# Desperodoo/distributed_multi_agent_reinforcement_learning

Hardware: AMD Instinct MI355X
Metric: env-steps/sec (whole node), pursuit-evasion 8-agent 4096-env (higher is better)
Workload: dtype f64 environment / f32 policy (f32 matrix products evaluated from exact 3-way bf16 operand splits, f32 accumulation and storage)

## Files before the change

distributed_multi_agent_reinforcement_learning_amd/csrc/mappo_split.hip:

```cpp
#include <hip/hip_runtime.h>
#include <stdint.h>
#include <string.h>

#include "mappo_ops.h"
#include "sb_gemm.hpp"
#include "sb_gru_seq.hpp"

extern "C" {

static int sb_gemm_any(int64_t R, int32_t N, int32_t K, const float *X, int64_t ldx, const float *W, int64_t ldw, const float *bias, int32_t relu,
                       const float *addend, int64_t lda, float *Y, int64_t ldy, uint8_t *ybits, int64_t ldyb, void *stream) {
    if (R < 0 || !X || !W || !Y || ldx < K || ldw < K || ldy < N || (addend && lda < N)) return MO_ERR_BAD_ARG;
    if ((ldx & 3) || (ldw & 3) || (ldy & 3) || (lda & 3) || ((uintptr_t)X & 15) || ((uintptr_t)W & 15) || ((uintptr_t)Y & 15) || ((uintptr_t)addend & 15) ||
        ((uintptr_t)bias & 15))
        return MO_ERR_BAD_ARG;
    if (R == 0) return 0;
    hipStream_t st = (hipStream_t)stream;
    if (N == 128 && K == 128) return launch_sb_gemm_best<4, 1>(R, X, ldx, W, ldw, bias, addend, lda, Y, ldy, relu, st, ybits, ldyb);
    if (N == 128 && K == 256) return launch_sb_gemm_best<8, 1>(R, X, ldx, W, ldw, bias, addend, lda, Y, ldy, relu, st, ybits, ldyb);
    if (ybits) return MO_ERR_BAD_ARG;
    if (N == 128 && K == 384) return launch_sb_gemm_best<12, 1>(R, X, ldx, W, ldw, bias, addend, lda, Y, ldy, relu, st);
    if (N == 256 && K == 128) return launch_sb_gemm_best<4, 2>(R, X, ldx, W, ldw, bias, addend, lda, Y, ldy, relu, st);
    if (N == 384 && K == 128) return launch_sb_gemm_best<4, 3>(R, X, ldx, W, ldw, bias, addend, lda, Y, ldy, relu, st);
    return MO_ERR_BAD_ARG;
}

int sb_gemm(int64_t R, int32_t N, int32_t K, const float *X, int64_t ldx, const float *W, int64_t ldw, const float *bias, int32_t relu,
            const float *addend, int64_t lda, float *Y, int64_t ldy, void *stream) {
    return sb_gemm_any(R, N, K, X, ldx, W, ldw, bias, relu, addend, lda, Y, ldy, nullptr, 0, stream);
}

int sb_gemm_signs(int64_t R, int32_t N, int32_t K, const float *X, int64_t ldx, const float *W, int64_t ldw, const float *bias, int32_t relu,
                  const float *addend, int64_t lda, float *Y, int64_t ldy, uint8_t *y_sign_bits, int64_t ld_bytes, void *stream) {
    if (!y_sign_bits || ld_bytes < N / 8) return MO_ERR_BAD_ARG;
    return sb_gemm_any(R, N, K, X, ldx, W, ldw, bias, relu, addend, lda, Y, ldy, y_sign_bits, ld_bytes, stream);
}

int64_t sb_gemm_masked_workspace(int32_t N) { return N > 0 ? (int64_t)1024 * N * 4 : 0; }

int sb_gemm_masked(int64_t R, int32_t N, int32_t K, const float *X, int64_t ldx, const float *W, int64_t ldw, const float *M, int64_t ldm,
                   int32_t mask_cols, float *Y, int64_t ldy, float *colsum, void *workspace, void *stream) {
    if (R < 0 || !X || !W || !M || !Y || !colsum || !workspace || ldx < K || ldw < K || ldy < N || ldm < N) return MO_ERR_BAD_ARG;
    if (mask_cols < 0 || mask_cols > N || (mask_cols & 127)) return MO_ERR_BAD_ARG;
    if ((ldx & 3) || (ldw & 3) || (ldy & 3) || (ldm & 3) || ((uintptr_t)X & 15) || ((uintptr_t)W & 15) || ((uintptr_t)Y & 15) || ((uintptr_t)M & 15) ||
        ((uintptr_t)colsum & 15) || ((uintptr_t)workspace & 15))
        return MO_ERR_BAD_ARG;
    hipStream_t st = (hipStream_t)stream;
    if (R == 0) return (int)hipMemsetAsync(colsum, 0, (size_t)N * 4, st);
    int dev = 0, cus = 256;
    if (hipGetDevice(&dev) == hipSuccess && hipDeviceGetAttribute(&cus, hipDeviceAttributeMultiprocessorCount, dev) != hipSuccess) cus = 256;
    if (cus > 512) return MO_ERR_BAD_ARG;
    float *part = (float *)workspace;
    const int mt = mask_cols / 128;
    if (N == 256 && K == 128) return launch_sb_gemm<4, 2, SBG_MASK_OPT_256>(R, X, ldx, W, ldw, nullptr, M, ldm, Y, ldy, 0, st, mt, part, colsum);
    if (N == 384 && K == 128) return launch_sb_gemm<4, 3, SBG_MASK_OPT_384>(R, X, ldx, W, ldw, nullptr, M, ldm, Y, ldy, 0, st, mt, part, colsum);
    if (N == 128 && K == 384) return launch_sb_gemm<12, 1, SBG_MASK_OPT_K384>(R, X, ldx, W, ldw, nullptr, M, ldm, Y, ldy, 0, st, mt, part, colsum);
    return MO_ERR_BAD_ARG;
}

int sb_gemm_masked_bits(int64_t R, int32_t N, int32_t K, const float *X, int64_t ldx, const float *W, int64_t ldw, const uint8_t *sign_bits,
                        int64_t ld_bytes, int32_t mask_cols, float *Y, int64_t ldy, float *colsum, void *workspace, void *stream) {
    if (R < 0 || !X || !W || !sign_bits || !Y || !colsum || !workspace || ldx < K || ldw < K || ldy < N || ld_bytes < N / 8) return MO_ERR_BAD_ARG;
    if (mask_cols < 0 || mask_cols > N || (mask_cols & 127)) return MO_ERR_BAD_ARG;
    if ((ldx & 3) || (ldw & 3) || (ldy & 3) || ((uintptr_t)X & 15) || ((uintptr_t)W & 15) || ((uintptr_t)Y & 15) || ((uintptr_t)colsum & 15) ||
        ((uintptr_t)workspace & 15))
        return MO_ERR_BAD_ARG;
    hipStream_t st = (hipStream_t)stream;
    if (R == 0) return (int)hipMemsetAsync(colsum, 0, (size_t)N * 4, st);
    int dev = 0, cus = 256;
    if (hipGetDevice(&dev) == hipSuccess && hipDeviceGetAttribute(&cus, hipDeviceAttributeMultiprocessorCount, dev) != hipSuccess) cus = 256;
    if (cus > 512) return MO_ERR_BAD_ARG;
    float *part = (float *)workspace;
    const float *m = (const float *)sign_bits;
    const int mt = mask_cols / 128;
    if (N == 256 && K == 128) return launch_sb_gemm<4, 2, SBG_MASK_OPT_256 | 16>(R, X, ldx, W, ldw, nullptr, m, ld_bytes, Y, ldy, 0, st, mt, part, colsum);
    if (N == 384 && K == 128) return launch_sb_gemm<4, 3, SBG_MASK_OPT_384 | 16>(R, X, ldx, W, ldw, nullptr, m, ld_bytes, Y, ldy, 0, st, mt, part, colsum);
    if (N == 128 && K == 384) return launch_sb_gemm<12, 1, SBG_MASK_OPT_K384 | 16>(R, X, ldx, W, ldw, nullptr, m, ld_bytes, Y, ldy, 0, st, mt, part, colsum);
    return MO_ERR_BAD_ARG;
}

int sb_gemm_n128(int64_t R, int32_t K, const float *X, int64_t ldx, const float *W, int64_t ldw, const float *bias, int32_t relu, const float *addend,
                 int64_t lda, float *Y, int64_t ldy, void *stream) {
    return sb_gemm(R, 128, K, X, ldx, W, ldw, bias, relu, addend, lda, Y, ldy, stream);
}

int gru_seq_split_fwd_multi(int32_t n_nets, const mo_gru_seq_net *nets, int32_t T, int32_t B, int32_t H, int32_t gi_agents, void *stream) {
    if (n_nets < 1 || n_nets > MO_GRU_MAX_NETS || !nets || T < 1 || B < 1 || H != SBR_H || gi_agents < 0 || (gi_agents && B % gi_agents)) return MO_ERR_BAD_ARG;
    for (int k = 0; k < n_nets; k++) {
        const mo_gru_seq_net &m = nets[k];
        if (!m.gi || !m.w_hh || !m.b_hh || !m.h0 || !m.out) return MO_ERR_BAD_ARG;
        if ((((uintptr_t)m.gi | (uintptr_t)m.w_hh | (uintptr_t)m.b_hh | (uintptr_t)m.h0 | (uintptr_t)m.out | (uintptr_t)m.save) & 15)) return MO_ERR_BAD_ARG;
        if (m.B < 0 || m.B > B || (gi_agents && m.B % gi_agents)) return MO_ERR_BAD_ARG;
    }
    return launch_gru_seq_fwd_sb(n_nets, nets, T, B, gi_agents, (hipStream_t)stream);
}

int gru_seq_split_bwd_multi(int32_t n_nets, const mo_gru_seq_bwd_net *nets, int32_t T, int32_t B, int32_t H, int32_t gi_agents, void *stream) {
    if (n_nets < 1 || n_nets > MO_GRU_MAX_NETS || !nets || T < 1 || B < 1 || H != SBR_H || gi_agents < 0 || (gi_agents && B % gi_agents)) return MO_ERR_BAD_ARG;
    for (int k = 0; k < n_nets; k++) {
        const mo_gru_seq_bwd_net &m = nets[k];
        if (!m.dout || !m.save || !m.out || !m.h0 || !m.w_hh || !m.dgi || !m.dh0) return MO_ERR_BAD_ARG;
        if ((m.dgh == nullptr) == (m.dnr == nullptr)) return MO_ERR_BAD_ARG;
        if ((m.db_ih || m.db_hh) && (!m.db_ih || !m.db_hh || !m.workspace)) return MO_ERR_BAD_ARG;
        if ((((uintptr_t)m.dout | (uintptr_t)m.save | (uintptr_t)m.out | (uintptr_t)m.h0 | (uintptr_t)m.dgi | (uintptr_t)m.dgh | (uintptr_t)m.dnr |
              (uintptr_t)m.dh0 | (uintptr_t)m.workspace) & 15)) return MO_ERR_BAD_ARG;
        if (m.B < 0 || m.B > B || (gi_agents && m.B % gi_agents)) return MO_ERR_BAD_ARG;
    }
    return launch_gru_seq_bwd_sb(n_nets, nets, T, B, gi_agents, (hipStream_t)stream);
}

}
```

include/mappo_ops.h:

```cpp
#ifndef MAPPO_OPS_H
#define MAPPO_OPS_H
#include <stdint.h>

#ifdef __cplusplus
extern "C" {
#endif

#define MO_ERR_BAD_ARG 20001

enum { MO_ADJ_TENSOR = 0,
       MO_ADJ_ONES = 1,
       MO_ADJ_VALID = 2,
       MO_ADJ_BITS = 3 };
#define MO_ADJ_ROW_WORDS(K) (((((K) + 31) >> 5) + 3) & ~3)

int dhgn_msg_agg_fwd(int32_t R, int32_t P, int32_t K, int32_t E, int32_t din, const float *p, int64_t p_row_stride,
                     const float *q, int64_t q_row_stride, int32_t q_div, const float *e, int64_t e_row_stride, const void *adj,
                     int64_t adj_row_stride, int32_t adj_mode, const int32_t *kvalid, const float *W, const float *b,
                     float *out, int64_t out_stride , void *stream);

typedef struct mo_msg_rel {
    int32_t K, din, q_div, adj_mode;
    const float *q; int64_t q_rs;
    const float *e; int64_t e_rs;
    const void *adj; int64_t adj_rs;
    const int32_t *kvalid;
    const float *W, *b;
} mo_msg_rel;
int dhgn_msg_agg3_fwd(const mo_msg_rel *rel , int32_t R, int32_t P, int32_t E, const float *p, int64_t p_row_stride, float *out,
                      int64_t out_stride, void *stream);
int dhgn_msg_agg3_pair_fwd(const mo_msg_rel *rel , int32_t R, int32_t P, int32_t E, const float *p, int64_t p_row_stride,
                           const int32_t *o_kvalid, float *out_actor, float *out_critic, int64_t out_stride, void *stream);

int dhgn_msg_agg3_pair01_fwd(const mo_msg_rel *rel , int32_t R, int32_t P, int32_t E, const float *p, int64_t p_row_stride,
                             float *out_actor, float *out_critic, int64_t out_stride, void *stream);
int dhgn_msg_agg_bwd_pair(int32_t R, int32_t P, int32_t K, int32_t E, int32_t din, const float *p, int64_t p_row_stride, const float *q,
                          int64_t q_row_stride, int32_t q_div, const float *e, int64_t e_row_stride, const float *adj, int64_t adj_row_stride,
                          const float *W, const float *b, const float *gout_actor, const float *gout_critic, int64_t gout_stride, float *dW,
                          float *db, void *workspace, void *stream);
int dhgn_msg_agg3_pair_pos_fwd(const mo_msg_rel *rel , int32_t R, int32_t P, int32_t E, const float *p, int64_t p_row_stride,
                               const int32_t *o_kvalid, float *out_actor, float *out_critic, int64_t out_stride, const float *Wp,
                               int64_t wp_row_stride, const float *bp, float *pos_actor, float *pos_critic, int64_t pos_stride, void *stream);

int64_t dhgn_msg_agg_bwd_workspace(int32_t E, int32_t din);
int dhgn_msg_agg_bwd(int32_t R, int32_t P, int32_t K, int32_t E, int32_t din, const float *p, int64_t p_row_stride,
                     const float *q, int64_t q_row_stride, int32_t q_div, const float *e, int64_t e_row_stride, const void *adj,
                     int64_t adj_row_stride, int32_t adj_mode, const int32_t *kvalid, const float *W, const float *b,
                     const float *gout, int64_t gout_stride, float *dW, float *db, void *workspace, void *stream);

int dhgn_msg_agg_ones_sorted_ok(int32_t R, int32_t P, int32_t K, int32_t E, int32_t din, int32_t q_div);
int64_t dhgn_msg_agg_ones_sorted_workspace(int32_t R, int32_t P, int32_t K, int32_t E, int32_t q_div, int64_t *m_bytes, int64_t *qtab_bytes,
                                           int64_t *partial_bytes);
int dhgn_msg_agg_ones_sorted_fwd(int32_t R, int32_t P, int32_t K, int32_t E, const float *p, int64_t p_row_stride, const float *q,
                                 int64_t q_row_stride, int32_t q_div, const float *W, const float *b, float *out, int64_t out_stride,
                                 uint8_t *save_m, float *qtab, void *stream);
int dhgn_msg_agg_ones_sorted_bwd(int32_t R, int32_t P, int32_t K, int32_t E, const float *p, int64_t p_row_stride, int32_t q_div,
                                 const float *gout, int64_t gout_stride, const uint8_t *save_m, const float *qtab, float *dW, float *db,
                                 void *partials, void *stream);

int64_t gae_advnorm_workspace(void);
int gae_advnorm(int32_t N, int32_t T, int32_t P, const float *r, const float *v, const float *active, float gamma,
                float lamda, int32_t use_adv_norm, float *adv, float *v_target, double *stats, void *stream);

int categorical_sample(int32_t R, int32_t A, const float *probs, uint64_t seed, uint64_t offset, int32_t greedy,
                       int32_t *action, float *logp, void *stream);
int categorical_sample_counter(int32_t R, int32_t A, const float *probs, uint64_t seed, uint64_t *counter, int32_t greedy,
                               int32_t *action, float *logp, void *stream);

int spectral_norm_weight(int32_t A, int32_t H, const float *W, float *u, float *v, float eps, int32_t n_power_iterations, float *w_eff,
                         void *stream);

int head_linear(int32_t R, int32_t A, int32_t H, const float *feat, const float *W, const float *b, float *y, void *stream);
int head_sample(int32_t R, int32_t A, int32_t H, const float *feat, const float *W, const float *b, uint64_t seed, uint64_t *counter,
                uint32_t *ticket, int32_t greedy, int32_t *action, float *logp, void *stream);

int gru_gates_fwd(int32_t B, int32_t H, const float *gi, const float *gh, const float *b_hh, const float *h_prev, float *h_out,
                  float *save, void *stream);
int gru_gates_bwd(int32_t B, int32_t H, const float *dout, const float *dcarry, const float *save, const float *h_prev, float *dgi,
                  float *dgh, float *dh_direct, void *stream);

int64_t gru_seq_save_elems(int32_t T, int32_t B);
#define MO_GRU_MAX_NETS 24
#define MO_GRU_CELL_MAX_NETS 4
typedef struct mo_gru_seq_net { const float *gi, *w_hh, *b_hh, *h0; float *out, *save; int32_t B, pad0; } mo_gru_seq_net;
typedef struct mo_gru_seq_bwd_net {
    const float *dout, *save, *out, *h0, *w_hh;
    float *dgi, *dgh, *dnr, *dh0, *db_ih, *db_hh;
    void *workspace;
    int32_t B, pad0;
} mo_gru_seq_bwd_net;
int gru_seq_fwd_multi(int32_t n_nets, const mo_gru_seq_net *nets, int32_t T, int32_t B, int32_t H, int32_t gi_agents, void *stream);
int gru_seq_bwd_multi(int32_t n_nets, const mo_gru_seq_bwd_net *nets, int32_t T, int32_t B, int32_t H, int32_t gi_agents, void *stream);
int gru_seq_split_fwd_multi(int32_t n_nets, const mo_gru_seq_net *nets, int32_t T, int32_t B, int32_t H, int32_t gi_agents, void *stream);
int gru_seq_split_bwd_multi(int32_t n_nets, const mo_gru_seq_bwd_net *nets, int32_t T, int32_t B, int32_t H, int32_t gi_agents, void *stream);
int gru_seq_fwd(int32_t T, int32_t B, int32_t H, const float *gi, const float *w_hh, const float *b_hh, const float *h0, float *out,
                float *save, int32_t gi_agents, void *stream);
int64_t gru_seq_bwd_workspace(int32_t B);
int gru_seq_bwd(int32_t T, int32_t B, int32_t H, const float *dout, const float *save, const float *out, const float *h0,
                const float *w_hh, float *dgi, float *dgh, float *dnr, float *dh0, float *db_ih, float *db_hh, int32_t gi_agents,
                void *workspace, void *stream);

int gru_cell_fwd(int32_t B, int32_t H, const float *x, const float *h_prev, const float *w_ih, const float *w_hh, const float *b_ih,
                 const float *b_hh, float *h_out, void *stream);
typedef struct mo_gru_cell_net { const float *x, *h_prev, *w_ih, *w_hh, *b_ih, *b_hh; float *h_out; } mo_gru_cell_net;
int gru_cell_fwd_multi(int32_t n_nets, const mo_gru_cell_net *nets, int32_t B, int32_t H, void *stream);
int gru_cell_split_fwd_multi(int32_t n_nets, const mo_gru_cell_net *nets, int32_t B, int32_t H, void *stream);
int sb_gemm_n128(int64_t R, int32_t K, const float *X, int64_t ldx, const float *W, int64_t ldw, const float *bias, int32_t relu, const float *C,
                 int64_t ldc, float *Y, int64_t ldy, void *stream);
int sb_gemm(int64_t R, int32_t N, int32_t K, const float *X, int64_t ldx, const float *W, int64_t ldw, const float *bias, int32_t relu, const float *C,
            int64_t ldc, float *Y, int64_t ldy, void *stream);
int sb_gemm_signs(int64_t R, int32_t N, int32_t K, const float *X, int64_t ldx, const float *W, int64_t ldw, const float *bias, int32_t relu, const float *C,
                  int64_t ldc, float *Y, int64_t ldy, uint8_t *y_sign_bits, int64_t ld_bytes, void *stream);
int64_t sb_gemm_masked_workspace(int32_t N);
int sb_gemm_masked(int64_t R, int32_t N, int32_t K, const float *X, int64_t ldx, const float *W, int64_t ldw, const float *M, int64_t ldm,
                   int32_t mask_cols, float *Y, int64_t ldy, float *colsum, void *workspace, void *stream);
int sb_gemm_masked_bits(int64_t R, int32_t N, int32_t K, const float *X, int64_t ldx, const float *W, int64_t ldw, const uint8_t *sign_bits,
                        int64_t ld_bytes, int32_t mask_cols, float *Y, int64_t ldy, float *colsum, void *workspace, void *stream);

int64_t ppo_loss_workspace(void);
int ppo_loss_fwd_bwd(int64_t n, const float *logp_now, const float *entropy, const float *logp_old, const float *adv, const float *active,
                     const float *values_now, const float *values_old, const float *v_target, const float *active_sum, float epsilon,
                     float entropy_coef, int32_t use_value_clip, float *losses, float *grad_logp, float *grad_entropy, float *grad_values,
                     void *workspace, void *stream);
int ppo_loss_prob_fwd_bwd(int64_t n, int32_t A, const float *prob, float *grad_prob, int64_t d1, int64_t d2, int64_t p_s0, int64_t p_s1, int64_t p_s2,
                          const float *action, const float *logp_old, const float *adv, const float *active, const float *values_now, int64_t v_s0,
                          int64_t v_s1, int64_t v_s2, const float *values_old, const float *v_target, const float *active_sum, float epsilon,
                          float entropy_coef, int32_t use_value_clip, float *losses, float *grad_values, void *workspace, void *stream);

int gauss_head_sample(int32_t R, int32_t A, int32_t H, const float *feat, const float *W, const float *b, const float *log_std, uint64_t seed,
                      uint64_t *counter, uint32_t *ticket, int32_t greedy, float *action, double *env_action, float *logp, void *stream);
int64_t ppo_loss_gauss_workspace(void);
int ppo_loss_gauss_fwd_bwd(int64_t n, int32_t A, const float *mu, float *grad_mu, int64_t d1, int64_t d2, int64_t m_s0, int64_t m_s1, int64_t m_s2,
                           const float *log_std, const float *action, const float *logp_old, const float *adv, const float *active,
                           const float *values_now, int64_t v_s0, int64_t v_s1, int64_t v_s2, const float *values_old, const float *v_target,
                           const float *active_sum, float epsilon, float entropy_coef, int32_t use_value_clip, float *losses, float *grad_values,
                           float *grad_log_std, void *workspace, void *stream);

#define MO_RECORD_MAX_ITEMS 16
typedef struct {
    const void *src;
    void *dst;
    int64_t dst_row_stride;
    int32_t row_bytes;
    int32_t i32_to_f32;
} mo_record_item;
int rollout_record(int32_t N, int32_t n_items, const mo_record_item *items, const float *raw, float *episode_return, int32_t P, void *stream);

int64_t wgrad_tn_workspace(int32_t M, int32_t N);
int wgrad_tn(int64_t K, int32_t M, int32_t N, const float *A, int64_t lda, const float *B, int64_t ldb, float *C, int32_t accumulate,
             void *workspace, void *stream);
int64_t wgrad_split_workspace(int32_t M, int32_t N);
int wgrad_split_tn(int64_t K, int32_t M, int32_t N, const float *A, int64_t lda, const float *B, int64_t ldb, float *C, int32_t accumulate,
                   void *workspace, void *stream);
int wgrad_split_tn2(int64_t K, int32_t M1, int32_t M2, int32_t N, const float *A1, int64_t lda1, const float *A2, int64_t lda2, const float *B, int64_t ldb,
                    float *C, int32_t accumulate, void *workspace, void *stream);
int fcra_neighbour_mean(int32_t R, int32_t P, int32_t E, int32_t T, const float *z_actor, int64_t za_episode_stride, int64_t za_step_stride,
                        const float *z_critic, int64_t zc_episode_stride, int64_t zc_step_stride, const float *adj, int64_t adj_row_stride,
                        const float *bias, int32_t relu, float *out_actor, float *out_critic, int64_t out_stride, void *stream);
#define MO_NBR_MAX_JOBS 4
typedef struct mo_nbr_job { const float *z_actor, *z_critic, *bias; float *out_actor, *out_critic; } mo_nbr_job;
int fcra_neighbour_mean_multi(int32_t n_jobs, const mo_nbr_job *jobs, int32_t R, int32_t P, int32_t E, int32_t T, int64_t za_episode_stride,
                              int64_t za_step_stride, int64_t zc_episode_stride, int64_t zc_step_stride, const float *adj, int64_t adj_row_stride,
                              int32_t relu, int64_t out_stride, void *stream);

int64_t relu_bwd_colsum_workspace(int32_t F);
int relu_bwd_colsum(int64_t R, int32_t F, const float *gout, int64_t g_row_stride, const float *y, int64_t y_row_stride, float *gin, float *colsum,
                    void *workspace, void *stream);

int64_t wgrad_skinny_workspace(int32_t NS, int32_t F);
int wgrad_skinny(int64_t R, int32_t NS, int32_t F, const float *S, int64_t lds, const float *X, int64_t ldx, int32_t transposed, float *C,
                 float *colsum_x, float *colsum_s, void *workspace, void *stream);

const char *mappo_ops_error_string(int code);

#ifdef __cplusplus
}
#endif
#endif
```

Measured before the change: 2.639 million.

## Add weight-stationary 32-row bf16-split GEMM kernel for masked 384-wide shapes

Adds a new persistent GEMM kernel that keeps the split bf16 weights in registers and streams 32-row input tiles through double-buffered shared memory, prefetching the next tile while the MFMAs run. It is enabled by default only for the masked (float-mask) 384-wide GEMMs at large row counts; other paths need an explicit selector call. The aim is to cut weight reloads and hide input latency, at the cost of high register pressure and a separate colsum reduction launch.

Result: no change. 2.638 million, median of 6 (-0.0%).

```diff
diff --git a/distributed_multi_agent_reinforcement_learning_amd/csrc/mappo_split.hip b/distributed_multi_agent_reinforcement_learning_amd/csrc/mappo_split.hip
--- a/distributed_multi_agent_reinforcement_learning_amd/csrc/mappo_split.hip
+++ b/distributed_multi_agent_reinforcement_learning_amd/csrc/mappo_split.hip
@@ -4,9 +4,20 @@
 
 #include "mappo_ops.h"
 #include "sb_gemm.hpp"
+#include "sb_gemm_w32.hpp"
 #include "sb_gru_seq.hpp"
 
+static constexpr int64_t SBW_MIN_ROWS = 131072;
+static int g_sbg_kernel = 0;
+static bool sbg_w32(int64_t R, bool by_default) { return g_sbg_kernel == 2 || (g_sbg_kernel == 0 && by_default && R >= SBW_MIN_ROWS); }
+
 extern "C" {
+
+int sb_gemm_select_kernel(int32_t which) {
+    if (which < 0 || which > 2) return MO_ERR_BAD_ARG;
+    g_sbg_kernel = which;
+    return 0;
+}
 
 static int sb_gemm_any(int64_t R, int32_t N, int32_t K, const float *X, int64_t ldx, const float *W, int64_t ldw, const float *bias, int32_t relu,
                        const float *addend, int64_t lda, float *Y, int64_t ldy, uint8_t *ybits, int64_t ldyb, void *stream) {
@@ -19,9 +30,17 @@
     if (N == 128 && K == 128) return launch_sb_gemm_best<4, 1>(R, X, ldx, W, ldw, bias, addend, lda, Y, ldy, relu, st, ybits, ldyb);
     if (N == 128 && K == 256) return launch_sb_gemm_best<8, 1>(R, X, ldx, W, ldw, bias, addend, lda, Y, ldy, relu, st, ybits, ldyb);
     if (ybits) return MO_ERR_BAD_ARG;
-    if (N == 128 && K == 384) return launch_sb_gemm_best<12, 1>(R, X, ldx, W, ldw, bias, addend, lda, Y, ldy, relu, st);
+    if (N == 128 && K == 384) {
+        if (sbg_w32(R, false)) return addend ? launch_sb_gemm_w32<12, 1, 1>(R, X, ldx, W, ldw, bias, addend, lda, Y, ldy, relu, st)
+                                      : launch_sb_gemm_w32<12, 1, 0>(R, X, ldx, W, ldw, bias, addend, lda, Y, ldy, relu, st);
+        return launch_sb_gemm_best<12, 1>(R, X, ldx, W, ldw, bias, addend, lda, Y, ldy, relu, st);
+    }
     if (N == 256 && K == 128) return launch_sb_gemm_best<4, 2>(R, X, ldx, W, ldw, bias, addend, lda, Y, ldy, relu, st);
-    if (N == 384 && K == 128) return launch_sb_gemm_best<4, 3>(R, X, ldx, W, ldw, bias, addend, lda, Y, ldy, relu, st);
+    if (N == 384 && K == 128) {
+        if (sbg_w32(R, false)) return addend ? launch_sb_gemm_w32<4, 3, 1>(R, X, ldx, W, ldw, bias, addend, lda, Y, ldy, relu, st)
+                                      : launch_sb_gemm_w32<4, 3, 0>(R, X, ldx, W, ldw, bias, addend, lda, Y, ldy, relu, st);
+        return launch_sb_gemm_best<4, 3>(R, X, ldx, W, ldw, bias, addend, lda, Y, ldy, relu, st);
+    }
     return MO_ERR_BAD_ARG;
 }
 
@@ -53,6 +72,10 @@
     float *part = (float *)workspace;
     const int mt = mask_cols / 128;
     if (N == 256 && K == 128) return launch_sb_gemm<4, 2, SBG_MASK_OPT_256>(R, X, ldx, W, ldw, nullptr, M, ldm, Y, ldy, 0, st, mt, part, colsum);
+    if (sbg_w32(R, true)) {
+        if (N == 384 && K == 128) return launch_sb_gemm_w32<4, 3, 4>(R, X, ldx, W, ldw, nullptr, M, ldm, Y, ldy, 0, st, mt, part, colsum);
+        if (N == 128 && K == 384) return launch_sb_gemm_w32<12, 1, 5>(R, X, ldx, W, ldw, nullptr, M, ldm, Y, ldy, 0, st, mt, part, colsum);
+    }
     if (N == 384 && K == 128) return launch_sb_gemm<4, 3, SBG_MASK_OPT_384>(R, X, ldx, W, ldw, nullptr, M, ldm, Y, ldy, 0, st, mt, part, colsum);
     if (N == 128 && K == 384) return launch_sb_gemm<12, 1, SBG_MASK_OPT_K384>(R, X, ldx, W, ldw, nullptr, M, ldm, Y, ldy, 0, st, mt, part, colsum);
     return MO_ERR_BAD_ARG;
@@ -74,6 +97,10 @@
     const float *m = (const float *)sign_bits;
     const int mt = mask_cols / 128;
     if (N == 256 && K == 128) return launch_sb_gemm<4, 2, SBG_MASK_OPT_256 | 16>(R, X, ldx, W, ldw, nullptr, m, ld_bytes, Y, ldy, 0, st, mt, part, colsum);
+    if (sbg_w32(R, false)) {
+        if (N == 384 && K == 128) return launch_sb_gemm_w32<4, 3, 20>(R, X, ldx, W, ldw, nullptr, m, ld_bytes, Y, ldy, 0, st, mt, part, colsum);
+        if (N == 128 && K == 384) return launch_sb_gemm_w32<12, 1, 20>(R, X, ldx, W, ldw, nullptr, m, ld_bytes, Y, ldy, 0, st, mt, part, colsum);
+    }
     if (N == 384 && K == 128) return launch_sb_gemm<4, 3, SBG_MASK_OPT_384 | 16>(R, X, ldx, W, ldw, nullptr, m, ld_bytes, Y, ldy, 0, st, mt, part, colsum);
     if (N == 128 && K == 384) return launch_sb_gemm<12, 1, SBG_MASK_OPT_K384 | 16>(R, X, ldx, W, ldw, nullptr, m, ld_bytes, Y, ldy, 0, st, mt, part, colsum);
     return MO_ERR_BAD_ARG;
diff --git a/distributed_multi_agent_reinforcement_learning_amd/csrc/sb_gemm_w32.hpp b/distributed_multi_agent_reinforcement_learning_amd/csrc/sb_gemm_w32.hpp
--- /dev/null
+++ b/distributed_multi_agent_reinforcement_learning_amd/csrc/sb_gemm_w32.hpp
@@ -0,0 +1,185 @@
+#pragma once
+#include <mutex>
+
+#include "sb_gemm.hpp"
+
+template <int KC, int NT, int OPT>
+__global__ __launch_bounds__(256) void k_sb_gemm_w32(int64_t R, const float *__restrict__ X, int64_t ldx, const float *__restrict__ W, int64_t ldw,
+                                                     const float *__restrict__ bias, const float *addend, int64_t lda, float *Y, int64_t ldy, int relu,
+                                                     int mask_tiles, float *__restrict__ colsum_part) {
+    static_assert(KC % 2 == 0 && KC * NT == 12, "the 384-wide shapes: 12 x 1 or 4 x 3");
+    extern __shared__ uint4 sbw_tile[];
+    constexpr int IMG = 3 * KC * 2 * 64, UPW = KC / 2, TPW = 2 * NT;
+    constexpr bool MASK = OPT & 4, BITS = (OPT & 4) && (OPT & 16), EARLY = (OPT & 1) && !BITS;
+    const int tid = threadIdx.x, w = tid >> 6, l = tid & 63, i = l & 15, gq = l >> 4;
+    uint4 wg[TPW][KC][3];
+#pragma unroll
+    for (int s = 0; s < TPW; s++) {
+        const float *rw = W + (size_t)(16 * (TPW * w + s) + i) * ldw + 8 * gq;
+#pragma unroll
+        for (int c = 0; c < KC; c++) sb_split8(*(const float4 *)(rw + 32 * c), *(const float4 *)(rw + 32 * c + 4), wg[s][c]);
+    }
+    const int64_t n_it = (R + 31) / 32;
+    float4 pf[UPW][2];
+    auto fetch1 = [&](int n, int64_t it) {
+        const int blk = w * UPW + n, c = blk >> 1, rt = blk & 1;
+        int64_t row = it * 32 + rt * 16 + i;
+        row = row < R ? row : R - 1;
+        const float *src = X + row * ldx + 32 * c + 8 * gq;
+        if constexpr (SBG_ABLATE & 4) {
+            pf[n][0] = pf[n][1] = make_float4((float)row * 1e-6f, 0.5f, -0.25f, (float)c);
+        } else {
+            pf[n][0] = *(const float4 *)src;
+            pf[n][1] = *(const float4 *)(src + 4);
+        }
+    };
+    auto stage1 = [&](int n, uint4 *img) {
+        const int blk = w * UPW + n;
+        uint4 p_[3];
+        sb_split8(pf[n][0], pf[n][1], p_);
+#pragma unroll
+        for (int p = 0; p < 3; p++) img[(p * KC * 2 + blk) * 64 + l] = p_[p];
+    };
+    int64_t it = blockIdx.x;
+#pragma unroll
+    for (int n = 0; n < UPW; n++) fetch1(n, it);
+#pragma unroll
+    for (int n = 0; n < UPW; n++) stage1(n, sbw_tile);
+#pragma unroll
+    for (int n = 0; n < UPW; n++) fetch1(n, it + gridDim.x);
+    lds_barrier();
+    int cur = 0;
+    float4 cs[TPW];
+#pragma unroll
+    for (int s = 0; s < TPW; s++) cs[s] = make_float4(0.f, 0.f, 0.f, 0.f);
+    for (; it < n_it; it += gridDim.x) {
+        const uint4 *tb = sbw_tile + cur * IMG + l;
+        uint4 *nimg = sbw_tile + (cur ^ 1) * IMG;
+        float4 a4[TPW][2];
+        unsigned mb[TPW][2];
+        if constexpr (EARLY) {
+#pragma unroll
+            for (int rt = 0; rt < 2; rt++) {
+                int64_t row = it * 32 + rt * 16 + i;
+                row = row < R ? row : R - 1;
+#pragma unroll
+                for (int s = 0; s < TPW; s++) a4[s][rt] = *(const float4 *)(addend + row * lda + 16 * (TPW * w + s) + 4 * gq);
+            }
+        }
+        f32x4 acc[TPW][2];
+#pragma unroll
+        for (int s = 0; s < TPW; s++) acc[s][0] = acc[s][1] = (f32x4){0.f, 0.f, 0.f, 0.f};
+        uint4 nb0[3], nb1[3];
+#pragma unroll
+        for (int p = 0; p < 3; p++) { nb0[p] = tb[(p * KC * 2) * 64]; nb1[p] = tb[(p * KC * 2 + 1) * 64]; }
+#pragma unroll
+        for (int c = 0; c < KC; c++) {
+            uint4 b0[3], b1[3];
+#pragma unroll
+            for (int p = 0; p < 3; p++) { b0[p] = nb0[p]; b1[p] = nb1[p]; }
+            if (c + 1 < KC) {
+#pragma unroll
+                for (int p = 0; p < 3; p++) { nb0[p] = tb[(p * KC * 2 + 2 * c + 2) * 64]; nb1[p] = tb[(p * KC * 2 + 2 * c + 3) * 64]; }
+            }
+            __builtin_amdgcn_sched_barrier(0);
+#define SBW_MMA(pi, pj)                                                                                                                             \
+            _Pragma("unroll") for (int s = 0; s < TPW; s++) {                                                                                         \
+                acc[s][0] = __builtin_amdgcn_mfma_f32_16x16x32_bf16(__builtin_bit_cast(bf16x8, wg[s][c][pi]), __builtin_bit_cast(bf16x8, b0[pj]), acc[s][0], 0, 0, 0); \
+                acc[s][1] = __builtin_amdgcn_mfma_f32_16x16x32_bf16(__builtin_bit_cast(bf16x8, wg[s][c][pi]), __builtin_bit_cast(bf16x8, b1[pj]), acc[s][1], 0, 0, 0); \
+            }
+            if constexpr (!(SBG_ABLATE & 1)) { SBW_MMA(2, 0) SBW_MMA(0, 2) SBW_MMA(1, 1) SBW_MMA(1, 0) SBW_MMA(0, 1) SBW_MMA(0, 0) }
+            else {
+#pragma unroll
+                for (int s = 0; s < TPW; s++) { acc[s][0][0] += __uint_as_float(b0[0].x ^ wg[s][c][0].x); acc[s][1][1] += __uint_as_float(b1[2].y ^ wg[s][c][2].w); }
+            }
+#undef SBW_MMA
+            if (!(c & 1)) {
+                stage1(c >> 1, nimg);
+                fetch1(c >> 1, it + 2 * (int64_t)gridDim.x);
+            }
+            __builtin_amdgcn_sched_barrier(0);
+        }
+        if constexpr (BITS) {
+            const uint8_t *bits = (const uint8_t *)addend;
+#pragma unroll
+            for (int rt = 0; rt < 2; rt++) {
+                int64_t row = it * 32 + rt * 16 + i;
+                row = row < R ? row : R - 1;
+#pragma unroll
+                for (int s = 0; s < TPW; s++)
+                    mb[s][rt] = ((TPW * w + s) >> 3) < mask_tiles ? (unsigned)bits[row * lda + 2 * (TPW * w + s) + (gq >> 1)] >> ((gq & 1) * 4) : 15u;
+            }
+        } else if constexpr (MASK && !EARLY) {
+#pragma unroll
+            for (int rt = 0; rt < 2; rt++) {
+                int64_t row = it * 32 + rt * 16 + i;
+                row = row < R ? row : R - 1;
+#pragma unroll
+                for (int s = 0; s < TPW; s++) a4[s][rt] = *(const float4 *)(addend + row * lda + 16 * (TPW * w + s) + 4 * gq);
+            }
+        }
+#pragma unroll
+        for (int rt = 0; rt < 2; rt++) {
+            const int64_t row = it * 32 + rt * 16 + i;
+            if (row < R) {
+#pragma unroll
+                for (int s = 0; s < TPW; s++) {
+                    const int g = TPW * w + s, col = 16 * g + 4 * gq;
+                    float4 v;
+                    if constexpr (MASK) {
+                        v = make_float4(acc[s][rt][0], acc[s][rt][1], acc[s][rt][2], acc[s][rt][3]);
+                        if constexpr (BITS) {
+                            const unsigned m = mb[s][rt];
+                            v.x = (m & 1u) ? v.x : 0.f; v.y = (m & 2u) ? v.y : 0.f; v.z = (m & 4u) ? v.z : 0.f; v.w = (m & 8u) ? v.w : 0.f;
+                        } else if ((g >> 3) < mask_tiles) {
+                            v.x = a4[s][rt].x > 0.f ? v.x : 0.f; v.y = a4[s][rt].y > 0.f ? v.y : 0.f;
+                            v.z = a4[s][rt].z > 0.f ? v.z : 0.f; v.w = a4[s][rt].w > 0.f ? v.w : 0.f;
+                        }
+                        cs[s].x += v.x; cs[s].y += v.y; cs[s].z += v.z; cs[s].w += v.w;
+                    } else {
+                        const float4 b4 = bias ? *(const float4 *)(bias + col) : make_float4(0.f, 0.f, 0.f, 0.f);
+                        v = make_float4(acc[s][rt][0] + b4.x, acc[s][rt][1] + b4.y, acc[s][rt][2] + b4.z, acc[s][rt][3] + b4.w);
+                        if (addend) {
+                            if constexpr (!EARLY) a4[s][rt] = *(const float4 *)(addend + row * lda + col);
+                            v.x += a4[s][rt].x; v.y += a4[s][rt].y; v.z += a4[s][rt].z; v.w += a4[s][rt].w;
+                        }
+                        if (relu) { v.x = fmaxf(v.x, 0.f); v.y = fmaxf(v.y, 0.f); v.z = fmaxf(v.z, 0.f); v.w = fmaxf(v.w, 0.f); }
+                    }
+                    if constexpr (SBG_ABLATE & 2) { if (v.x == 12345.678f) *(float4 *)(Y + row * ldy + col) = v; }
+                    else *(float4 *)(Y + row * ldy + col) = v;
+                }
+            }
+        }
+        lds_barrier();
+        cur ^= 1;
+    }
+    if constexpr (MASK) {
+#pragma unroll
+        for (int s = 0; s < TPW; s++) {
+#pragma unroll
+            for (int m = 1; m < 16; m <<= 1) {
+                cs[s].x += __shfl_xor(cs[s].x, m); cs[s].y += __shfl_xor(cs[s].y, m);
+                cs[s].z += __shfl_xor(cs[s].z, m); cs[s].w += __shfl_xor(cs[s].w, m);
+            }
+            if (i == 0) *(float4 *)(colsum_part + (size_t)blockIdx.x * (128 * NT) + 16 * (TPW * w + s) + 4 * gq) = cs[s];
+        }
+    }
+}
+
+template <int KC, int NT, int OPT>
+int launch_sb_gemm_w32(int64_t R, const float *X, int64_t ldx, const float *W, int64_t ldw, const float *bias, const float *addend, int64_t lda,
+                       float *Y, int64_t ldy, int relu, hipStream_t st, int mask_tiles = 0, float *colsum_part = nullptr, float *colsum = nullptr) {
+    constexpr int lds = 2 * 3 * KC * 2 * 64 * 16;
+    static std::once_flag once;
+    static hipError_t attr_rc = hipSuccess;
+    std::call_once(once, [] { attr_rc = hipFuncSetAttribute((const void *)k_sb_gemm_w32<KC, NT, OPT>, hipFuncAttributeMaxDynamicSharedMemorySize, lds); });
+    if (attr_rc != hipSuccess) return (int)attr_rc;
+    int dev = 0, cus = 256;
+    if (hipGetDevice(&dev) == hipSuccess && hipDeviceGetAttribute(&cus, hipDeviceAttributeMultiprocessorCount, dev) != hipSuccess) cus = 256;
+    const int64_t n_it = (R + 31) / 32;
+    const int grid = n_it < (int64_t)cus ? (int)n_it : cus;
+    hipLaunchKernelGGL((k_sb_gemm_w32<KC, NT, OPT>), dim3(grid), dim3(256), lds, st, R, X, ldx, W, ldw, bias, addend, lda, Y, ldy, relu, mask_tiles,
+                       colsum_part);
+    if constexpr (OPT & 4) hipLaunchKernelGGL(k_sb_colsum_reduce, dim3(NT), dim3(128), 0, st, grid, 128 * NT, colsum_part, colsum);
+    return (int)hipGetLastError();
+}
diff --git a/include/mappo_ops.h b/include/mappo_ops.h
--- a/include/mappo_ops.h
+++ b/include/mappo_ops.h
@@ -116,6 +116,7 @@
                    int32_t mask_cols, float *Y, int64_t ldy, float *colsum, void *workspace, void *stream);
 int sb_gemm_masked_bits(int64_t R, int32_t N, int32_t K, const float *X, int64_t ldx, const float *W, int64_t ldw, const uint8_t *sign_bits,
                         int64_t ld_bytes, int32_t mask_cols, float *Y, int64_t ldy, float *colsum, void *workspace, void *stream);
+int sb_gemm_select_kernel(int32_t which);
 
 int64_t ppo_loss_workspace(void);
 int ppo_loss_fwd_bwd(int64_t n, const float *logp_now, const float *entropy, const float *logp_old, const float *adv, const float *active,
```
